# groupeLIAMG/ttcr

Hardware: AMD Instinct MI355X
Metric: Mnodes/s per sweep-iteration (512^3 fp32 grid, first-order FSM) (higher is better)
Workload: dtype f32

## Files before the change

### include/ttcr_amd.h

```cpp
#ifndef TTCR_AMD_H
#define TTCR_AMD_H

#include <stddef.h>
#include <stdint.h>

#ifdef __cplusplus
extern "C" {
#endif

typedef struct ttcr_fsm_grid ttcr_fsm_grid;

enum { TTCR_F32 = 0, TTCR_F64 = 1 };

enum {
    TTCR_OK = 0,
    TTCR_ERR_VALUE = 1,
    TTCR_ERR_RUNTIME = 2,
    TTCR_ERR_DEVICE = 3,
    TTCR_ERR_UNSUPPORTED = 4
};

int ttcr_fsm_device_count(void);

const char* ttcr_fsm_last_error(void);
// ... 200 lines not shown
    double total_ms;
    long long kernel_launches;
    long long node_updates;
    long long evaluated_updates;
    int iterations;
    int n_sources;
} ttcr_fsm_timing;
int ttcr_fsm_last_timing(const ttcr_fsm_grid* g, ttcr_fsm_timing* out);
int ttcr_fsm_stopping_stats(const ttcr_fsm_grid* g, long long* reference_sums, long long* reference_sums_missed, long long* rounds);
int ttcr_fsm_prefill_swaps(const ttcr_fsm_grid* g, long long* swaps);
int ttcr_fsm_prefill_inline_fills(const ttcr_fsm_grid* g, long long* fills);
int ttcr_fsm_reference_change(ttcr_fsm_grid* g, const void* times, const void* field, int parallel, void* out);
int ttcr_fsm_last_kernel(const ttcr_fsm_grid* g, char* buf, size_t n);
int ttcr_fsm_unit_order(int dim, int dtype, int stage, int by_time, uint32_t nnx, uint32_t nny, uint32_t nnz, uint32_t* out,
                        size_t capacity, size_t* n_units);
int ttcr_fsm_prefill_slice(int dtype, uint64_t n_el, uint32_t n_tickets, uint32_t ticket, uint64_t* slice_len, uint64_t* begin, uint64_t* end);
const char* ttcr_fsm_build_id(void);

#ifdef __cplusplus
}
#endif
#endif
```

### ttcr_amd/_lib.py

```python
import ctypes as C
import os

HERE = os.path.dirname(os.path.abspath(__file__))
LIB_PATH = os.environ.get("TTCR_AMD_LIB") or os.path.join(HERE, "libttcr_amd.so")

TTCR_F32, TTCR_F64 = 0, 1
OK, ERR_VALUE, ERR_RUNTIME, ERR_DEVICE, ERR_UNSUPPORTED = 0, 1, 2, 3, 4

_P = C.c_void_p
_U32 = C.c_uint32
_D = C.c_double
_I = C.c_int


class Timing(C.Structure):
    _fields_ = [("sweep_ms", C.c_double), ("total_ms", C.c_double), ("kernel_launches", C.c_longlong),
                ("node_updates", C.c_longlong), ("evaluated_updates", C.c_longlong), ("iterations", C.c_int),
                ("n_sources", C.c_int)]


SYMBOLS = {
    "ttcr_fsm_device_count": (_I, []),
    "ttcr_fsm_last_error": (C.c_char_p, []),
    "ttcr_fsm3d_create": (_I, [C.POINTER(_P), _I, _I, _U32, _U32, _U32, _D, _D, _D, _D, _D, _I, _I, _I, _I, _I]),
# ... 15 lines not shown
    "ttcr_fsm_compute_slowness": (_I, [_P, _I, _P, _I, _P]),
    "ttcr_fsm_get_niter": (_I, [_P, _I, C.POINTER(_I), C.POINTER(_I)]),
    "ttcr_fsm_get_changes": (_I, [_P, _I, C.POINTER(_D), _I, C.POINTER(_D), _I]),
    "ttcr_fsm_get_reference_changes": (_I, [_P, _I, C.POINTER(_D), _I, C.POINTER(_D), _I]),
    "ttcr_fsm_n_slots": (_I, [_P]),
    "ttcr_fsm_n_nodes": (C.c_size_t, [_P]),
    "ttcr_fsm_n_cells": (C.c_size_t, [_P]),
    "ttcr_fsm_set_option": (_I, [_P, C.c_char_p, _D]),
    "ttcr_fsm_last_timing": (_I, [_P, C.POINTER(Timing)]),
    "ttcr_fsm_last_kernel": (_I, [_P, C.c_char_p, C.c_size_t]),
    "ttcr_fsm_build_id": (C.c_char_p, []),
    "ttcr_fsm_unit_order": (_I, [_I, _I, _I, _I, _U32, _U32, _U32, C.POINTER(_U32), C.c_size_t, C.POINTER(C.c_size_t)]),
    "ttcr_fsm_stopping_stats": (_I, [_P, C.POINTER(C.c_longlong), C.POINTER(C.c_longlong), C.POINTER(C.c_longlong)]),
    "ttcr_fsm_prefill_swaps": (_I, [_P, C.POINTER(C.c_longlong)]),
    "ttcr_fsm_prefill_inline_fills": (_I, [_P, C.POINTER(C.c_longlong)]),
    "ttcr_fsm_prefill_slice": (_I, [_I, C.c_uint64, _U32, _U32, C.POINTER(C.c_uint64), C.POINTER(C.c_uint64), C.POINTER(C.c_uint64)]),
    "ttcr_fsm_reference_change": (_I, [_P, C.c_void_p, C.c_void_p, C.c_int, C.c_void_p]),
    "ttcr_fsm_rays_size": (_I, [_P, C.POINTER(C.c_size_t), C.POINTER(C.c_size_t)]),
    "ttcr_fsm_get_rays": (_I, [_P, _P, _P]),
    "ttcr_fsm_raytrace_rays": (_I, [_P, _I, _I, _P, _P, _I, _P, _P]),
    "ttcr_fsm_slot_rays_size": (_I, [_P, _I, C.POINTER(C.c_size_t), C.POINTER(C.c_size_t)]),
    "ttcr_fsm_get_slot_rays": (_I, [_P, _I, _P, _P]),
    "ttcr_fsm_raytrace_m": (_I, [_P, _I, _I, _P, _P, _I, _P, _P]),
    "ttcr_fsm_raytrace_rm": (_I, [_P, _I, _I, _P, _P, _I, _P, _P]),
    "ttcr_fsm_raytrace_multi_m": (_I, [_P, _I, _P, _P, _P, _P, _P, _P, _I]),
    "ttcr_fsm_multi_m_size": (_I, [_P, C.POINTER(C.c_size_t), C.POINTER(C.c_size_t)]),
    "ttcr_fsm_get_multi_m": (_I, [_P, _P, _P, _P]),
    "ttcr_fsm_raytrace_multi_tape": (_I, [_P, _I, _P, _P, _P, _P, _P, _P, C.POINTER(_P)]),
    "ttcr_fsm_tape_size": (_I, [_P, C.POINTER(C.c_size_t), C.POINTER(C.c_size_t), C.POINTER(C.c_size_t)]),
    "ttcr_fsm_tape_bytes": (_I, [_P, C.POINTER(C.c_size_t)]),
# ... 134 lines not shown
```

### ttcr_amd/build.py

```python
import os
import shutil
import subprocess

HERE = os.path.dirname(os.path.abspath(__file__))
CSRC = os.path.join(HERE, "csrc")
OBJ = os.path.join(CSRC, "_obj")
LIB = os.path.join(HERE, "libttcr_amd.so")
INC = os.path.join("..", "..", "include", "ttcr_amd.h")
UNITS = {
    "fsm_capi.hip": ([], ["fsm_capi.hip", "fsm_kernels.h", "fsm_fast_api.h", "fsm_march_levels.inc", "fsm_fast.hip", "fsm_tape_api.h",
                          "fsm_tape.hip", "fsm_adjoint_api.h", "fsm_adjoint.hip", "fsm_normal.hip", "fsm_locate.hip", "fsm_model.hip", "fsm_unit_order.h", "fsm_prefill_slices.h", INC]),
    "fsm_fast.hip": ([], ["fsm_fast.hip", "fsm_fast_api.h", "fsm_kernels.h", "fsm_march_levels.inc", "fsm_prefill_slices.h"]),
    "fsm_tape.hip": ([], ["fsm_tape.hip", "fsm_tape_api.h"]),
    "fsm_adjoint.hip": ([], ["fsm_adjoint.hip", "fsm_adjoint_api.h", "fsm_kernels.h", "fsm_march_levels.inc", "fsm_prefill_slices.h"]),
    "fsm_normal.hip": ([], ["fsm_normal.hip", "fsm_adjoint_api.h"]),
    "fsm_locate.hip": ([], ["fsm_locate.hip", "fsm_adjoint_api.h"]),
    "fsm_model.hip": ([], ["fsm_model.hip", "fsm_adjoint_api.h"]),
}
SOURCES = list(UNITS)
DEPS = sorted({d for _, ds in UNITS.values() for d in ds})
FLAGS = ["--offload-arch=gfx950", "-O3", "-std=c++17", "-fPIC", "-ffp-contract=off",
         "-fno-fast-math", "-Wall", "-Wno-unused-result"]


def _hipcc():
    for c in (os.environ.get("HIPCC"), shutil.which("hipcc"), "/opt/rocm/bin/hipcc"):
        if c and os.path.exists(c):
            return c
    raise RuntimeError("hipcc not found")
# ... 53 lines not shown
```

### ttcr_amd/csrc/fsm_capi.hip

```cpp
#include <hip/hip_runtime.h>

#include <algorithm>
#include <atomic>
#include <chrono>
#include <condition_variable>
#include <cmath>
#include <cstdio>
#include <cstdlib>
#include <cstring>
#include <limits>
#include <map>
#include <memory>
#include <mutex>
#include <sstream>
#include <stdexcept>
#include <string>
#include <thread>
#include <vector>

#include "../../include/ttcr_amd.h"
#include "fsm_kernels.h"
#include "fsm_fast_api.h"
#include "fsm_tape_api.h"
#include "fsm_adjoint_api.h"
#include "fsm_unit_order.h"

#ifndef FSM_CHUNK3
#define FSM_CHUNK3 8
#endif

namespace ttcr_amd {

static thread_local std::string g_last_error;

struct ValueError : std::runtime_error {
    using std::runtime_error::runtime_error;
};
struct DeviceError : std::runtime_error {
    using std::runtime_error::runtime_error;
};
// ... 253 lines not shown
    size_t ssh_stride = 0;
    DevBuf<uint32_t> d_mask;
    DevBuf<int> d_bbox, d_slots, d_lmask;
    int* h_lmask = nullptr;
    DevBuf<uint32_t> d_tiles;
    std::vector<int> tile_off, tile_cnt;
    DevBuf<double> d_change;
    DevBuf<unsigned long long> d_prof;
    size_t prof_words = 0;
    DevBuf<uint32_t> d_order;
    DevBuf<uint32_t> d_order_xs[2][2];
    DevBuf<int> d_sync;
    int n_patches = 0;
    int* h_abort = nullptr;
    DevBuf<int> d_stamp;
    DevBuf<unsigned long long> d_cmap;
    int cmap_words = 1;
    DevBuf<unsigned long long> d_sw;
    int sw_sweeps = 0;
    DevBuf<int> d_iter;
    DevBuf<unsigned long long> d_evals;
    int* h_iter = nullptr;
    unsigned launch_epoch = 1;
    bool sync_clean = true;
    size_t sync_words = 0;
    unsigned long long* h_evals = nullptr;
    int nbf = 0, nbj = 0, nbk = 0;
    size_t n_bricks = 0;
    DevBuf<InitPoint<T>> d_pts;
    double* h_change = nullptr;
// ... 108 lines not shown
        HIP_CHECK(hipMemsetAsync(d_ssh.p, 0, ssh_stride * (dim == 3 ? 4 : 2) * sizeof(T), stream));
        if (dim == 3) build_tile_lists(TileCfg<T, 3>::PJ, TileCfg<T, 3>::PK, TileCfg<T, 3>::BL);
        else build_tile_lists(TileCfg<T, 2>::PJ, TileCfg<T, 2>::PK, TileCfg<T, 2>::BL);
        build_persistent_lists();
        nbf = (geom.NF + FSM_BRICK - 1) / FSM_BRICK;
        nbj = (geom.NJ + FSM_BRICK - 1) / FSM_BRICK;
        nbk = (geom.NK + FSM_BRICK - 1) / FSM_BRICK;
        n_bricks = (size_t)nbf * nbj * nbk;
        d_stamp.reserve(n_bricks * n_slots);
        {
            const int PJ = dim == 3 ? TileCfg<T, 3>::PJ : TileCfg<T, 2>::PJ, PK = dim == 3 ? TileCfg<T, 3>::PK : 1;
            const int max_chunks = (geom.NF + 2 * (PJ + PK)) / 4 + 4;
            cmap_words = max_chunks / 32 + 1;
            d_cmap.reserve((size_t)n_patches * n_slots * (dim == 3 ? 8 : 4) * 2 * cmap_words);
            HIP_CHECK(hipMemset(d_cmap.p, 0, (size_t)n_patches * n_slots * (dim == 3 ? 8 : 4) * 2 * cmap_words * sizeof(unsigned long long)));
            sw_sweeps = (dim == 3 ? 8 : 4) * (2 * std::min(nitermax, 256) + 2);
            d_sw.reserve((size_t)sw_sweeps * n_slots);
        }
        d_iter.reserve(2);
        d_evals.reserve(n_slots);
        if (dim == 2)
            HIP_CHECK(hipFuncSetAttribute(reinterpret_cast<const void*>(&fsm_sweep45_rows<T>),
                                          hipFuncAttributeMaxDynamicSharedMemorySize, 156 * 1024));
        if (const char* e = std::getenv("TTCR_FSM_SWEEP45")) sweep45_strips = std::string(e) == "strips";
        if (const char* e = std::getenv("TTCR_FSM_WENO_CH4_MIN")) weno_ch4_min = std::atoi(e);
        if (const char* e = std::getenv("TTCR_FSM_WENO_C16_BELOW")) weno_c16_below = std::atoi(e);
        if (const char* e = std::getenv("TTCR_FSM_F64_C16_BELOW")) f64_c16_below = std::atoi(e);
        if (const char* e = std::getenv("TTCR_FSM_TIME_ORDER_BELOW")) time_order_below = std::atoi(e);
        if (const char* e = std::getenv("TTCR_FSM_PRE_MIN")) pre_min = std::atoi(e);
        if (const char* e = std::getenv("TTCR_FSM_SKIP")) skip = std::atoi(e);
// ... 73 lines not shown
        a.w = 0;
        a.variant = DIM == 3 ? 0 : (dx == dz ? 1 : 2);
        pa.order = d_order.p;
        pa.sync = d_sync.p;
        pa.n_patches = n_patches;
        pa.batch = batch;
        pa.timeout_ticks = 300000000ull;
        pa.stamp = d_stamp.p;
        pa.iter_ptr = d_iter.p;
        pa.evals = d_evals.p;
        pa.nbf = nbf; pa.nbj = nbj; pa.nbk = nbk;
        pa.ndir = DIM == 3 ? 8 : 4;
        pa.skip = skip_now(batch) ? (std::getenv("TTCR_FSM_SKIP_ALL_DIRTY") ? 2 : 1) : 0;
        pa.cmap = d_cmap.p;
        pa.cw = cmap_words;
        pa.sw = std::getenv("TTCR_FSM_NO_SW") ? nullptr : d_sw.p;
        pa.n_sw_groups = n_groups();
        pa.n_sw_sweeps = sw_sweeps;
        pa.fill_dst = nullptr;
        pa.fill_slice = 0;
        pa.fill_n = 0;

        const size_t wg_cap = (fsm_looped(DIM == 3, H) && persist_wgs > 0) ? (size_t)persist_wgs : ~(size_t)0;
        const dim3 block(C::PJ * C::PK), grid((unsigned)std::min<size_t>((size_t)n_patches * batch, wg_cap));
        const int ndir = DIM == 3 ? 8 : 4;
        {
            const bool pre_ = mode == 2 && !NO_PRE && (DIM == 2 || batch >= pre_min || dyn_lds > 0);
            char nm[160];
            std::snprintf(nm, sizeof nm, "fsm_sweep_persistent<%s,%d,%d,%d,%s,%s,%d,%d,%s,%s>", sizeof(T) == 4 ? "float" : "double", C::PJ, C::PK, CH,
                          DIM == 3 ? "true" : "false", skip_now(batch) ? "true" : "false", H, NSV, mode == 2 ? "true" : "false", pre_ ? "true" : "false");
// ... 327 lines not shown
                if (tile_cnt[w] == 0) continue;
                a.w = w;
                a.tiles = d_tiles.p + tile_off[w];
                const dim3 grid(tile_cnt[w], 1, batch);
                fsm_sweep_tile<T, C::PJ, C::PK, C::BL, DIM == 3><<<grid, block, 0, stream>>>(a);
            }
        }
        last_kernel = std::string("fsm_sweep_tile<") + (sizeof(T) == 4 ? "float" : "double") + "," + std::to_string(C::PJ) + "," + std::to_string(C::PK) + "," + std::to_string(C::BL) + "," + (DIM == 3 ? "true" : "false") + ">";
        HIP_CHECK(hipGetLastError());
    }

    int NS = 1;
    bool ns_window = false;
    int pair_layout = -1;
    double last_eval_frac = -1;
    double layout_lo = 0.55, layout_hi = 0.70;
    void choose_layout() {
        if (!ns_window) return;
        int want = NS;
        if (pair_layout >= 0) want = pair_layout ? 2 : 1;
        else if (last_eval_frac >= 0) want = NS == 2 ? (last_eval_frac < layout_lo ? 1 : 2) : (last_eval_frac > layout_hi ? 2 : 1);
        if (want == NS) return;
        NS = want;
        graph_batches[0] = graph_batches[1] = -1;
        for (int q = 0; q < n_slots; ++q) phys[q] = q;
    }
    int n_groups() const { return (n_slots + NS - 1) / NS; }
    size_t tt_fields() const { return (size_t)n_slots + ((ns_window || NS == 2) ? (size_t)(n_slots & 1) : 0); }
    T* tt_ptr(int slot) const { return d_tt.p + (size_t)(slot / NS) * n_nodes * NS + slot % NS; }
    template <int H>
    bool fast_now() const { return sizeof(T) == 4 && (arith == 2 || (arith == 1 && !weno)); }
// ... 19 lines not shown
    int skip_probe_min = 1024;
    bool probe_skip = true;
    int probe_off_calls = 0;
    int persist_wgs = 2048;
    bool in_probe_window(int entries) const {
        const long long u = (long long)n_patches * entries;
        return dim == 3 && sizeof(T) == 4 && u >= skip_probe_min && u < skip_units_min;
    }
    int skip_default(int entries) const {
        if (dim != 3) return 1;
        if (stage == 1) return 1;
        if (in_probe_window(entries)) return probe_skip ? 1 : 0;
        return (long long)n_patches * entries >= skip_units_min ? 1 : 0;
    }
    bool persistent_now() const { return mode >= 1 || stage == 1; }
    bool skip_now(int entries) const {
        const int on = skip < 0 ? skip_default(entries) : skip;
        const bool fits = (long long)geom.NF + geom.NJ + geom.NK < (1ll << 22) && nbf <= 32 * FSM_SLAB_WORDS;
        return on != 0 && fits && !(dim == 2 && rotated && !weno && dx == dz);
    }

    void launch_sweep45(int batch) {
        Sweep45Args<T> a;
        a.tt = d_tt.p;
        a.s = d_s.p;
        a.frozen = d_mask.p;
        a.change = d_change.p;
        a.slots = d_slots.p;
        a.lmask = d_lmask.p;
        a.ts = NS;
        a.by_group = persistent_now() ? 1 : 0;
        a.nnx = (int)ncx + 1;
        a.nnz = (int)ncz + 1;
// ... 436 lines not shown

        const int maxit = fixed_iters > 0 ? fixed_iters : nitermax;
        const int ndir = dim == 3 ? 8 : 4;
        if (!sync_clean || launch_epoch > 0xfffff000u) {
            HIP_CHECK(hipMemsetAsync(d_sync.p, 0, sync_words * sizeof(int), stream));
            HIP_CHECK(hipMemsetAsync(d_cmap.p, 0, (size_t)n_patches * n_slots * ndir * 2 * cmap_words * sizeof(unsigned long long), stream));
            HIP_CHECK(hipStreamSynchronize(stream));
            launch_epoch = 1;
        }
        sync_clean = false;
        snap_always = false;
        if (persistent_now() || weno) HIP_CHECK(hipMemsetAsync(d_sync.p + 8, 0, (sync_words - 8) * sizeof(int), stream));
        if (persistent_now() || weno) HIP_CHECK(hipMemsetAsync(d_sync.p + 4, 0, sizeof(int), stream));
        HIP_CHECK(hipMemsetAsync(d_evals.p, 0, sizeof(unsigned long long) * n_slots, stream));
        HIP_CHECK(hipMemsetAsync(d_sw.p, 0, sizeof(unsigned long long) * (size_t)sw_sweeps * n_groups(), stream));
        HIP_CHECK(hipEventRecord(ev0, stream));
        int it_total = 0;
        for (stage = 0; stage < (weno ? 2 : 1); ++stage) {
            std::vector<int> active(slot_ids);
            int it = 0;
            prev_change.assign(n_slots, std::numeric_limits<double>::infinity());
            prev2_change.assign(n_slots, std::numeric_limits<double>::infinity());
            snap_iter.assign(n_groups(), 0);
            snap_T.assign(n_groups(), -1);
            stamps_ok = false;
            if ((int)ref_change_last.size() != n_slots) ref_change_last.assign(n_slots, std::nan(""));
            std::vector<int> groups;
            for (int s2 : slot_ids)
                if (groups.empty() || groups.back() != s2 / NS) groups.push_back(s2 / NS);
            while (!active.empty() && it < maxit) {
// ... 3200 lines not shown
        } else {
            PJ = dim == 3 ? TileCfg<double, 3>::PJ : TileCfg<double, 2>::PJ; PK = dim == 3 ? TileCfg<double, 3>::PK : 1;
            C = dim == 3 ? ChunkCfg<double, 3>::C : ChunkCfg<double, 2>::C;
        }
        const uint64_t npj = ((uint64_t)NJ + PJ - 1) / PJ, npk = ((uint64_t)NK + PK - 1) / PK;
        if (NF >= (1u << 30) || npj >= (1u << 14) || npk >= (1u << 14)) throw ValueError("grid too large for the patch index of the sweep kernel");
        *n_units = (size_t)(npj * npk) * (dim == 3 ? 8 : 4);
        if (!out) return;
        if (capacity < *n_units) throw ValueError("output buffer too small for the units of the launch");
        const std::vector<uint32_t> xs = fsm_xs_order(dim, (int)NF, (int)NJ, (int)NK, PJ, PK, C, stage == 0 ? 1 : 2, by_time != 0,
                                                      fsm_diag_order((int)npj, (int)npk));
        std::copy(xs.begin(), xs.end(), out);
    });
}

int ttcr_fsm_prefill_slice(int dtype, uint64_t n_el, uint32_t n_tickets, uint32_t ticket, uint64_t* slice_len, uint64_t* begin, uint64_t* end) {
    return guarded([&] {
        if (dtype != TTCR_F32 && dtype != TTCR_F64) throw ValueError("dtype must be TTCR_F32 or TTCR_F64");
        if (n_tickets == 0) throw ValueError("a launch has at least one ticket");
        const size_t slice = fsm_fill_slice_len((size_t)n_el, n_tickets, dtype == TTCR_F32 ? 4 : 2);
        size_t b = 0, e = 0;
        fsm_fill_slice_range((size_t)n_el, slice, ticket, &b, &e);
        if (slice_len) *slice_len = slice;
        if (begin) *begin = b;
        if (end) *end = e;
    });
}

const char* ttcr_fsm_build_id(void) { return TTCR_BUILD_ID; }

// ... 2 lines not shown
```

### ttcr_amd/csrc/fsm_kernels.h

```cpp
#pragma once
#include <hip/hip_runtime.h>
#include <stdint.h>
#include <type_traits>

#include "fsm_prefill_slices.h"

namespace ttcr_amd {

constexpr int FSM_BRICK = 16;

template <typename T> struct real_traits;
template <> struct real_traits<float> {
    static __host__ __device__ constexpr float max() { return 3.402823466e+38f; }
    static __device__ __forceinline__ float inf() { return __builtin_huge_valf(); }
};
template <> struct real_traits<double> {
    static __host__ __device__ constexpr double max() { return 1.7976931348623157e+308; }
    static __device__ __forceinline__ double inf() { return __builtin_huge_val(); }
};

__device__ __forceinline__ uint32_t idx_u32(double v) { return v < 0 ? 0u : (v >= 4294967295.0 ? 4294967295u : (uint32_t)v); }

__device__ __forceinline__ float rmin(float a, float b) { return a < b ? a : b; }
__device__ __forceinline__ double rmin(double a, double b) { return a < b ? a : b; }
// ... 405 lines not shown
    SweepArgs<T> s;
    const uint32_t* order;
    int* sync;
    int n_patches, batch;
    unsigned long long timeout_ticks;
    int* stamp;
    const int* iter_ptr;
    unsigned long long* evals;
    int nbf, nbj, nbk;
    int dir, ndir;
    int skip;
    unsigned long long* cmap;
    int cw;
    unsigned long long* sw;
    int n_sw_groups, n_sw_sweeps;
    const T* ssh;
    size_t ssh_stride;
    T* fill_dst;
    size_t fill_slice;
    size_t fill_n;
};



__device__ __forceinline__ float ld_sc1(const float* p) {
    return __uint_as_float(__hip_atomic_load((const unsigned int*)p, __ATOMIC_RELAXED, __HIP_MEMORY_SCOPE_AGENT));
}
__device__ __forceinline__ double ld_sc1(const double* p) {
    return __longlong_as_double(__hip_atomic_load((const long long*)p, __ATOMIC_RELAXED, __HIP_MEMORY_SCOPE_AGENT));
}
// ... 238 lines not shown
    const float disc3 = __builtin_fmaf(3.0f * fh, fh, -(df2 + __builtin_fmaf(d3, d3, e * e)));
    const float t3 = __builtin_fmaf(1.0f / 3.0f, (d3 - df) + __builtin_amdgcn_sqrtf(disc3), a1);
    return t1 > a2 ? (t2 > a3 ? t3 : t2) : t1;
}

#ifndef FSM_POLL_SLEEP
#define FSM_POLL_SLEEP 2
#endif
#ifndef FSM_MINW
#define FSM_MINW 1
#endif
#ifndef FSM_SLAB_WORDS
#define FSM_SLAB_WORDS 32
#endif
#define FSM_FIN 0x3ffffff0
#ifndef FSM_SKIP_ABL
#define FSM_SKIP_ABL 0
#endif
#ifndef FSM_EARLY_PUB
#define FSM_EARLY_PUB 0
#endif
__device__ __forceinline__ float lane_below(float x, float edge) {
    return __uint_as_float((unsigned)__builtin_amdgcn_update_dpp((int)__float_as_uint(edge), (int)__float_as_uint(x), 0x138, 0xf, 0xf, false));
}
__device__ __forceinline__ float lane_above(float x, float edge) {
    return __uint_as_float((unsigned)__builtin_amdgcn_update_dpp((int)__float_as_uint(edge), (int)__float_as_uint(x), 0x130, 0xf, 0xf, false));
}
__device__ __forceinline__ double lane_below(double x, double edge) {
    const unsigned long long u = (unsigned long long)__double_as_longlong(x), e = (unsigned long long)__double_as_longlong(edge);
    const unsigned lo = (unsigned)__builtin_amdgcn_update_dpp((int)(unsigned)e, (int)(unsigned)u, 0x138, 0xf, 0xf, false);
// ... 39 lines not shown
    const unsigned long long u = (unsigned long long)__float_as_uint(x.v[0]) | ((unsigned long long)__float_as_uint(x.v[1]) << 32);
    __hip_atomic_store((unsigned long long*)p, u, __ATOMIC_RELAXED, __HIP_MEMORY_SCOPE_AGENT);
}
__device__ __forceinline__ void st_sc1(Pack<double, 2>* p, Pack<double, 2> x) {
    st_sc1(&p->v[0], x.v[0]);
    st_sc1(&p->v[1], x.v[1]);
}

__host__ __device__ constexpr bool fsm_looped(bool is3d, int h) { return is3d && h == 1; }

__device__ __forceinline__ int kmaxp_of(int k0, int NK, int PK) { return (k0 + PK < NK ? k0 + PK : NK) - 1; }
template <typename T, int PJ, int PK, int C, bool IS3D, bool SKIP, int H, int NS, bool XS, bool PRE, int AR = 0>
__device__ __forceinline__ bool fsm_sweep_unit(const PersistArgs<T>& pa) {
    static_assert(AR == 0 || std::is_same<T, float>::value, "tolerance-grade arithmetic: fp32 kernels");
    constexpr bool LOOPED = fsm_looped(IS3D, H);
    using P = Pack<T, NS>;
    constexpr int NT = PJ * PK;
    constexpr int RJ = PJ + 2 * H;
    constexpr int NROWS = IS3D ? RJ * (PK + 2 * H) : RJ;
    constexpr int NQ = C + 2 * H;
    constexpr int RS = NQ | 1;
    constexpr int NUP = IS3D ? H * (PJ + PK) : H;
    constexpr int NDH = IS3D ? H * (PJ + PK) : H;
    constexpr int RPI = NT / C;
    constexpr int NOWN = C;
    constexpr int NHI = (NDH + RPI - 1) / RPI;
    constexpr int NUPI = (NUP + RPI - 1) / RPI;
    static_assert(NT % C == 0 && (IS3D || PK == 1) && C <= FSM_BRICK && (H == 1 || H == 2), "tile shape");
    static_assert(C - 1 <= FSM_XPAD, "the rows of a chunk are read from the sheared copies without a wrap");
    static_assert(!(SKIP && FSM_EARLY_PUB > 0), "FSM_EARLY_PUB is a tuning option of the kernels without exact skipping");
// ... 7 lines not shown
        __hip_atomic_store(p_, (int)(((unsigned)e2 << 30) | (unsigned)v_), __ATOMIC_RELAXED, __HIP_MEMORY_SCOPE_AGENT);
    };
    auto ld_cmap = [&](const unsigned long long* p_) -> unsigned {
        const unsigned long long v_ = __hip_atomic_load(p_, __ATOMIC_RELAXED, __HIP_MEMORY_SCOPE_AGENT);
        return (unsigned)(v_ >> 32) == epoch ? (unsigned)v_ : 0u;
    };
    auto st_cmap = [&](unsigned long long* p_, unsigned v_) {
        __hip_atomic_store(p_, ((unsigned long long)epoch << 32) | v_, __ATOMIC_RELAXED, __HIP_MEMORY_SCOPE_AGENT);
    };

    __shared__ P Tt[NROWS * RS];
    __shared__ int s_ticket, s_abort;
    __shared__ int s_anychg;
    constexpr int SLABW = SKIP ? FSM_SLAB_WORDS : 1;
    __shared__ unsigned s_stamped[SKIP ? 9 : 1][SLABW];
    __shared__ unsigned s_slab[SLABW];
    __shared__ int s_next, s_act;
    __shared__ int s_cwi[2], s_cwl[2];
    __shared__ unsigned s_cwv[2];
    __shared__ int s_mywi;
    __shared__ unsigned s_mywv[2];
    enum { U_THR, U_RSJLO, U_RSKLO, U_RSNJ, U_RSNK, U_LCF, U_UPLCF0, U_UPLCF1, U_HIST, U_EVER, U_UCHG, U_PENDV, U_LCHG, U_N };
    __shared__ int s_u[U_N];

    int tid = threadIdx.x;
    if constexpr (LOOPED) asm volatile("" : "+v"(tid));
    unsigned long long prof_t = (FSM_ENABLE_PROF && a.prof) ? wall_clock64() : 0ull;
    unsigned long long pacc[6] = {0, 0, 0, 0, 0, 0};
    unsigned pchunks = 0;
    unsigned long long twait = 0;
    constexpr int FSM_TRACE_UNITS = FSM_ENABLE_PROF == 2 ? (1 << 20) : 65536;
    const unsigned long long trace_t0 = prof_t;
    unsigned long long* prec = nullptr;
    __shared__ unsigned long long s_pacc[FSM_ENABLE_PROF == 2 ? 8 : 1];
    if constexpr (FSM_ENABLE_PROF == 2) {
        if (tid == 0) {
            for (int q = 0; q < 6; ++q) s_pacc[q] = 0;
            s_pacc[6] = prof_t;
// ... 368 lines not shown
                        if (__hip_atomic_load(pa.sync + 4, __ATOMIC_RELAXED, __HIP_MEMORY_SCOPE_AGENT)) break;
                        if (wall_clock64() - t0 > pa.timeout_ticks) {
                            __hip_atomic_store(pa.sync + 4, 1, __ATOMIC_RELAXED, __HIP_MEMORY_SCOPE_AGENT);
                            break;
                        }
                    }
                    __builtin_amdgcn_s_sleep(8);
                }
            }
        }
        __syncthreads();
    }
    if (CHASE_OK && chase) chase_wait(Lc - C, -1, false);
    if (!SKIP) { issue_static(Lc); pref_for = Lc; }
    if constexpr (SKIP) {
        const int nsw = (pa.nbf + 31) >> 5;
        for (int w = tid; w < nsw; w += NT) s_slab[w] = 0u;
        for (int w = tid; w < 9 * SLABW; w += NT) s_stamped[w / SLABW][w % SLABW] = 0u;
        if (tid == 0) {
            s_cwi[0] = -1; s_cwi[1] = -1; s_mywi = -1;
            const int ja = j0 - H < 0 ? 0 : j0 - H, jb = jmaxp + H > NJ - 1 ? NJ - 1 : jmaxp + H;
            const int ka = k0 - H < 0 ? 0 : k0 - H, kb = kmaxp + H > NK - 1 ? NK - 1 : kmaxp + H;
            const int jlo = (rj ? NJ - 1 - jb : ja) / FSM_BRICK, jhi = (rj ? NJ - 1 - ja : jb) / FSM_BRICK;
            const int klo = (rk ? NK - 1 - kb : ka) / FSM_BRICK, khi = (rk ? NK - 1 - ka : kb) / FSM_BRICK;
            s_u[U_RSJLO] = jlo; s_u[U_RSNJ] = jhi - jlo + 1;
            s_u[U_RSKLO] = klo; s_u[U_RSNK] = khi - klo + 1;
            const int sg = pa.ndir * pa.iter_ptr[0] + dir + 1;
            s_u[U_THR] = pa.skip == 2 ? -(1 << 30) : (sg - 1 > 0 ? sg - 1 : 0);
            s_u[U_LCF] = Lc;
            const int lsj = Ls - PJ, lsk = Ls - PK, mu = TJ + TK - 1;
            s_u[U_UPLCF0] = lsj - (((lsj - mu) % C + C) % C);
            s_u[U_UPLCF1] = lsk - (((lsk - mu) % C + C) % C);
            s_u[U_HIST] = 0; s_u[U_EVER] = 0; s_u[U_UCHG] = 0; s_u[U_PENDV] = 0; s_u[U_LCHG] = 0;
        }
        __syncthreads();
        {
            const int jlo = s_u[U_RSJLO], nj = s_u[U_RSNJ], klo = s_u[U_RSKLO], nk = s_u[U_RSNK], thr = s_u[U_THR];
            const int* __restrict__ stamp = pa.stamp + (size_t)grp * pa.nbf * pa.nbj * pa.nbk;
            const int total = pa.nbf * nj * nk;
            for (int b = tid; b < total; b += NT) {
                const int bf = b % pa.nbf, jk = b / pa.nbf;
                const int bj = jlo + jk % nj, bk = klo + jk / nj;
                const int v = __hip_atomic_load(stamp + ((size_t)bk * pa.nbj + bj) * pa.nbf + bf, __ATOMIC_RELAXED, __HIP_MEMORY_SCOPE_AGENT);
                if (v >= thr) atomicOr(&s_slab[bf >> 5], 1u << (bf & 31));
            }
        }
        __syncthreads();
    }
    FSM_PMARK(5)
    const unsigned long long trace_t1 = (FSM_ENABLE_PROF && a.prof) ? wall_clock64() : 0ull;
    auto cmap_of = [&](int pidx, int e) -> unsigned long long* {
// ... 80 lines not shown
                        const int need8 = (L + C - 1) << 8;
                        bool ok = true;
                        if (up_j && pre_j < need8) pre_j = poll_until(up_j, need8, ok);
                        if (up_k && ok && pre_k < need8) pre_k = poll_until(up_k, need8, ok);
                        if (!ok) act = 0;
                        break;
                    }
                    const int need = L + C - 1, need8 = need << 8;
                    int vj = FSM_FIN, vk = FSM_FIN;
                    bool ok = true;
                    if (up_j) { vj = pre_j >= need8 ? pre_j : poll_until(up_j, need8, ok); pre_j = vj; }
                    if (up_k && ok) { vk = pre_k >= need8 ? pre_k : poll_until(up_k, need8, ok); pre_k = vk; }
                    if (!ok) { act = 0; break; }
                    if (L == lcf && vj >= FSM_FIN && !(vj & 1) && vk >= FSM_FIN && !(vk & 2)) {
                        bool any = false;
                        for (int w = 0; w < ((pa.nbf + 31) >> 5); ++w) any |= s_slab[w] != 0u;
                        if (!any) {
                            st_prog(my_prog, FSM_FIN);
                            L = Le + 1;
                            act = 0;
                            break;
                        }
                    }
                    int flo, fhi;
                    chunk_frange(L, H, flo, fhi);
                    bool dirty = slab_any(flo, fhi);
                    if (!dirty && up_j) dirty = up_dirty(vj, need, 0);
                    if (!dirty && up_k) dirty = up_dirty(vk, need, 1);
                    if (dirty) break;
                    if (pending) { act = 2; break; }
                    L += C;
                    h = (h << 2) & 0xff;
                    if (L > Le && s_u[U_UCHG]) {
                        s_u[U_PENDV] = FSM_FIN | s_u[U_EVER];
                    } else {
                        st_prog(my_prog, L > Le ? (FSM_FIN | s_u[U_EVER]) : ((L << 8) | h));
                    }
                }
                s_u[U_HIST] = h;
                s_next = L;
                s_act = act;
// ... 176 lines not shown
        FSM_PMARK(3)
        if (FSM_ENABLE_PROF) ++pchunks;

        if constexpr (SKIP) {
            const bool ej = changed && jp + H > jmaxp, ek = IS3D && changed && kp + H > kmaxp;
            const int f = (wave_any(changed) ? 1 : 0) | (wave_any(ej) ? 2 : 0) | (wave_any(ek) ? 4 : 0);
            if (f && (tid & 63) == 0) atomicOr(&s_anychg, f);
            if (!(FSM_SKIP_ABL & 2) && changed) {
                const int ip0 = L0 - jp - kp;
                const int ia = ip0 + ea, ib = ip0 + eb;
                const int ba = (rf ? NF - 1 - ib : ia) / FSM_BRICK, bb2 = (rf ? NF - 1 - ia : ib) / FSM_BRICK;
                const int my_bj = (rj ? NJ - 1 - jp : jp) / FSM_BRICK - s_u[U_RSJLO], my_bk = (rk ? NK - 1 - kp : kp) / FSM_BRICK - s_u[U_RSKLO];
                const int jk = my_bk * s_u[U_RSNJ] + my_bj;
                atomicOr(&s_stamped[jk][ba >> 5], 1u << (ba & 31));
                if (bb2 != ba) atomicOr(&s_stamped[jk][bb2 >> 5], 1u << (bb2 & 31));
            }
        } else {
            if (wave_any(changed) && (tid & 63) == 0) s_anychg = 1;
        }
        __syncthreads();
        const int chg_flags = SKIP ? __builtin_amdgcn_readfirstlane(s_anychg) : s_anychg;
        const bool any_changed = chg_flags != 0;
        if (any_changed) {
#pragma unroll
            for (int it = 0; it < NOWN; ++it) {
                const int ipm = L0 + ipb[it] - H;
                if ((unsigned)ipm < (unsigned)NF) {
                    const int rid = rsub + RPI * it;
                    const int cj = rid % PJ, ck = rid / PJ;
                    P* dst = Tg + (abase[it] + sf * (L0 - H));
                    const P v = Tt[lrow[it] - H];
                    if (XS || cj >= PJ - H || (IS3D && ck >= PK - H)) st_sc1(dst, v); else *dst = v;
                }
            }
        }
        if constexpr (SKIP) {
            if (!(FSM_SKIP_ABL & 4) && tid == 0) {
                if (any_changed) {
                    int flo, fhi;
                    chunk_frange(L0, 0, flo, fhi);
                    for (int b = flo / FSM_BRICK; b <= fhi / FSM_BRICK; ++b) s_slab[b >> 5] |= 1u << (b & 31);
                    const int ci = (L0 - s_u[U_LCF]) / C, w = ci >> 5;
                    if ((chg_flags & 6) && w < pa.cw) {
                        if (s_mywi != w) { s_mywi = w; s_mywv[0] = 0u; s_mywv[1] = 0u; }
                        for (int e2 = 0; e2 < 2; ++e2)
                            if (chg_flags & (2 << e2)) {
                                s_mywv[e2] |= 1u << (ci & 31);
                                st_cmap(cmap_of(TK * npj + TJ, e2) + w, s_mywv[e2]);
                            }
                    }
                    s_u[U_UCHG] = 1;
                    s_u[U_LCHG] = 1;
                }
                const int h2 = ((s_u[U_HIST] << 2) | (chg_flags >> 1)) & 0xff, ev2 = s_u[U_EVER] | (chg_flags >> 1);
                s_u[U_HIST] = h2;
                s_u[U_EVER] = ev2;
                s_u[U_PENDV] = Lc + C > Le ? (FSM_FIN | ev2) : (((Lc + C) << 8) | h2);
            }
        }
// ... 8 lines not shown
        ++n_done;
        FSM_PMARK(4)
    }
    if constexpr (SKIP) {
        __syncthreads();
        if (s_u[U_UCHG]) {
            const int nsw = (pa.nbf + 31) >> 5;
            const int rs_jlo = s_u[U_RSJLO], rs_nj = s_u[U_RSNJ], rs_klo = s_u[U_RSKLO], njk = rs_nj * s_u[U_RSNK];
            int* __restrict__ stamp = pa.stamp + (size_t)grp * pa.nbf * pa.nbj * pa.nbk;
            const int sigma = pa.ndir * pa.iter_ptr[0] + dir + 1;
            for (int q = tid; q < njk * nsw * 32; q += NT) {
                const int jk = q / (nsw * 32), bf = q % (nsw * 32);
                if (bf < pa.nbf && ((s_stamped[jk][bf >> 5] >> (bf & 31)) & 1u))
                    atomicMax(stamp + ((size_t)(rs_klo + jk / rs_nj) * pa.nbj + rs_jlo + jk % rs_nj) * pa.nbf + bf, sigma);
            }
            pending = 1;
        }
    }
    if (pending) {
        asm volatile("s_waitcnt vmcnt(0)" ::: "memory");
        __syncthreads();
        if (tid == 0) st_prog(my_prog, SKIP ? s_u[U_PENDV] : pending);
    }
    if constexpr (SKIP) {
        const int sigma0 = pa.ndir * pa.iter_ptr[0] + dir;
        if (tid == 0 && pa.sw && sigma0 < pa.n_sw_sweeps)
            atomicAdd(pa.sw + (size_t)sigma0 * pa.n_sw_groups + grp, 1ull | (s_u[U_UCHG] ? (1ull << 32) : 0ull));
    }

    if (FSM_ENABLE_PROF && a.prof && tid == 0) {
// ... 22 lines not shown
    for (int l = 0; l < NS; ++l) {
        double accd = (double)dec[l];
#pragma unroll
        for (int off = 32; off > 0; off >>= 1) accd += __shfl_down(accd, off, 64);
        if ((tid & 63) == 0 && accd != 0.0) atomicAdd(a.change + grp * NS + l, accd);
        if ((tid & 63) == 0 && nevals && ((lm >> l) & 1)) atomicAdd(pa.evals + grp * NS + l, nevals);
    }
    return true;
}

template <typename T, int PJ, int PK, int C, bool IS3D, bool SKIP, int H, int NS, bool XS, bool PRE = false, int AR = 0>
#ifndef FSM_WENO_MINW
#define FSM_WENO_MINW FSM_MINW
#endif
__global__ __launch_bounds__(PJ* PK, (SKIP && IS3D && H == 1 && NS == 2 && sizeof(T) == 4) ? 3
                                     : (IS3D && H == 2 && NS == 1 && sizeof(T) == 4) ? FSM_WENO_MINW : FSM_MINW) void fsm_sweep_persistent(const PersistArgs<T> pa) {
    if constexpr (fsm_looped(IS3D, H)) {
        (void)pa;
        for (;;) {
            auto kp = __builtin_amdgcn_kernarg_segment_ptr();
            asm volatile("" : "+s"(kp));
            if (!fsm_sweep_unit<T, PJ, PK, C, IS3D, SKIP, H, NS, XS, PRE, AR>(*(const PersistArgs<T>*)kp)) break;
        }
    } else {
        fsm_sweep_unit<T, PJ, PK, C, IS3D, SKIP, H, NS, XS, PRE, AR>(pa);
    }
}

template <typename T>
struct Sweep45Args {
// ... 1772 lines not shown
```

Measured before the change: 95910.

## Track per-chunk dirty bits for next sweep direction instead of brick slab scan

Adds a per-patch, per-direction chunk dirty bitmap. Each tile writes the chunks of neighbouring tiles that its updated nodes affect in the next sweep direction, and reads its own bitmap to decide which level chunks to skip. This replaces the per-chunk scan of brick stamps and slab bits with a single bit lookup, and also retunes the layout switch thresholds. In exchange it adds shared-memory arrays, atomic ORs to global memory, and extra register pressure, with a lower occupancy bound for the fp64 variant.

```diff
diff --git a/include/ttcr_amd.h b/include/ttcr_amd.h
--- a/include/ttcr_amd.h
+++ b/include/ttcr_amd.h
@@ -238,6 +238,7 @@
 int ttcr_fsm_last_kernel(const ttcr_fsm_grid* g, char* buf, size_t n);
 int ttcr_fsm_unit_order(int dim, int dtype, int stage, int by_time, uint32_t nnx, uint32_t nny, uint32_t nnz, uint32_t* out,
                         size_t capacity, size_t* n_units);
+int ttcr_fsm_chunk_dirty_marks(int dtype, int chunk, int dir, int edge_rule, uint32_t nnx, uint32_t nny, uint32_t nnz, int32_t* out, size_t capacity);
 int ttcr_fsm_prefill_slice(int dtype, uint64_t n_el, uint32_t n_tickets, uint32_t ticket, uint64_t* slice_len, uint64_t* begin, uint64_t* end);
 const char* ttcr_fsm_build_id(void);
 
diff --git a/ttcr_amd/_lib.py b/ttcr_amd/_lib.py
--- a/ttcr_amd/_lib.py
+++ b/ttcr_amd/_lib.py
@@ -53,6 +53,7 @@
     "ttcr_fsm_stopping_stats": (_I, [_P, C.POINTER(C.c_longlong), C.POINTER(C.c_longlong), C.POINTER(C.c_longlong)]),
     "ttcr_fsm_prefill_swaps": (_I, [_P, C.POINTER(C.c_longlong)]),
     "ttcr_fsm_prefill_inline_fills": (_I, [_P, C.POINTER(C.c_longlong)]),
+    "ttcr_fsm_chunk_dirty_marks": (_I, [_I, _I, _I, _I, _U32, _U32, _U32, C.POINTER(C.c_int32), C.c_size_t]),
     "ttcr_fsm_prefill_slice": (_I, [_I, C.c_uint64, _U32, _U32, C.POINTER(C.c_uint64), C.POINTER(C.c_uint64), C.POINTER(C.c_uint64)]),
     "ttcr_fsm_reference_change": (_I, [_P, C.c_void_p, C.c_void_p, C.c_int, C.c_void_p]),
     "ttcr_fsm_rays_size": (_I, [_P, C.POINTER(C.c_size_t), C.POINTER(C.c_size_t)]),
diff --git a/ttcr_amd/build.py b/ttcr_amd/build.py
--- a/ttcr_amd/build.py
+++ b/ttcr_amd/build.py
@@ -9,10 +9,10 @@
 INC = os.path.join("..", "..", "include", "ttcr_amd.h")
 UNITS = {
     "fsm_capi.hip": ([], ["fsm_capi.hip", "fsm_kernels.h", "fsm_fast_api.h", "fsm_march_levels.inc", "fsm_fast.hip", "fsm_tape_api.h",
-                          "fsm_tape.hip", "fsm_adjoint_api.h", "fsm_adjoint.hip", "fsm_normal.hip", "fsm_locate.hip", "fsm_model.hip", "fsm_unit_order.h", "fsm_prefill_slices.h", INC]),
-    "fsm_fast.hip": ([], ["fsm_fast.hip", "fsm_fast_api.h", "fsm_kernels.h", "fsm_march_levels.inc", "fsm_prefill_slices.h"]),
+                          "fsm_tape.hip", "fsm_adjoint_api.h", "fsm_adjoint.hip", "fsm_normal.hip", "fsm_locate.hip", "fsm_model.hip", "fsm_unit_order.h", "fsm_prefill_slices.h", "fsm_chunk_dirty.h", INC]),
+    "fsm_fast.hip": ([], ["fsm_fast.hip", "fsm_fast_api.h", "fsm_kernels.h", "fsm_march_levels.inc", "fsm_prefill_slices.h", "fsm_chunk_dirty.h"]),
     "fsm_tape.hip": ([], ["fsm_tape.hip", "fsm_tape_api.h"]),
-    "fsm_adjoint.hip": ([], ["fsm_adjoint.hip", "fsm_adjoint_api.h", "fsm_kernels.h", "fsm_march_levels.inc", "fsm_prefill_slices.h"]),
+    "fsm_adjoint.hip": ([], ["fsm_adjoint.hip", "fsm_adjoint_api.h", "fsm_kernels.h", "fsm_march_levels.inc", "fsm_prefill_slices.h", "fsm_chunk_dirty.h"]),
     "fsm_normal.hip": ([], ["fsm_normal.hip", "fsm_adjoint_api.h"]),
     "fsm_locate.hip": ([], ["fsm_locate.hip", "fsm_adjoint_api.h"]),
     "fsm_model.hip": ([], ["fsm_model.hip", "fsm_adjoint_api.h"]),
diff --git a/ttcr_amd/csrc/fsm_capi.hip b/ttcr_amd/csrc/fsm_capi.hip
--- a/ttcr_amd/csrc/fsm_capi.hip
+++ b/ttcr_amd/csrc/fsm_capi.hip
@@ -24,6 +24,7 @@
 #include "fsm_tape_api.h"
 #include "fsm_adjoint_api.h"
 #include "fsm_unit_order.h"
+#include "fsm_chunk_dirty.h"
 
 #ifndef FSM_CHUNK3
 #define FSM_CHUNK3 8
@@ -307,6 +308,7 @@
     int n_patches = 0;
     int* h_abort = nullptr;
     DevBuf<int> d_stamp;
+    DevBuf<unsigned> d_cdirty;
     DevBuf<unsigned long long> d_cmap;
     int cmap_words = 1;
     DevBuf<unsigned long long> d_sw;
@@ -445,6 +447,8 @@
             cmap_words = max_chunks / 32 + 1;
             d_cmap.reserve((size_t)n_patches * n_slots * (dim == 3 ? 8 : 4) * 2 * cmap_words);
             HIP_CHECK(hipMemset(d_cmap.p, 0, (size_t)n_patches * n_slots * (dim == 3 ? 8 : 4) * 2 * cmap_words * sizeof(unsigned long long)));
+            cdirty_wpu = ((geom.NF + 2 * (PJ + PK)) / 8 + 4) / 32 + 1;
+            if (dim == 3) d_cdirty.reserve(cdirty_words());
             sw_sweeps = (dim == 3 ? 8 : 4) * (2 * std::min(nitermax, 256) + 2);
             d_sw.reserve((size_t)sw_sweeps * n_slots);
         }
@@ -548,6 +552,8 @@
         pa.skip = skip_now(batch) ? (std::getenv("TTCR_FSM_SKIP_ALL_DIRTY") ? 2 : 1) : 0;
         pa.cmap = d_cmap.p;
         pa.cw = cmap_words;
+        pa.cdirty = d_cdirty.p;
+        pa.cdw = cdirty_wpu;
         pa.sw = std::getenv("TTCR_FSM_NO_SW") ? nullptr : d_sw.p;
         pa.n_sw_groups = n_groups();
         pa.n_sw_sweeps = sw_sweeps;
@@ -905,7 +911,7 @@
     bool ns_window = false;
     int pair_layout = -1;
     double last_eval_frac = -1;
-    double layout_lo = 0.55, layout_hi = 0.70;
+    double layout_lo = 0.45, layout_hi = 0.55;
     void choose_layout() {
         if (!ns_window) return;
         int want = NS;
@@ -955,9 +961,11 @@
         return (long long)n_patches * entries >= skip_units_min ? 1 : 0;
     }
     bool persistent_now() const { return mode >= 1 || stage == 1; }
+    int cdirty_wpu = 1;
+    size_t cdirty_words() const { return (size_t)n_patches * n_slots * 8 * cdirty_wpu; }
     bool skip_now(int entries) const {
         const int on = skip < 0 ? skip_default(entries) : skip;
-        const bool fits = (long long)geom.NF + geom.NJ + geom.NK < (1ll << 22) && nbf <= 32 * FSM_SLAB_WORDS;
+        const bool fits = (long long)geom.NF + geom.NJ + geom.NK < (1ll << 22) && nbf <= 32 * FSM_SLAB_WORDS && (dim != 3 || cdirty_wpu <= FSM_CD_WORDS);
         return on != 0 && fits && !(dim == 2 && rotated && !weno && dx == dz);
     }
 
@@ -1424,6 +1432,7 @@
         if (persistent_now() || weno) HIP_CHECK(hipMemsetAsync(d_sync.p + 4, 0, sizeof(int), stream));
         HIP_CHECK(hipMemsetAsync(d_evals.p, 0, sizeof(unsigned long long) * n_slots, stream));
         HIP_CHECK(hipMemsetAsync(d_sw.p, 0, sizeof(unsigned long long) * (size_t)sw_sweeps * n_groups(), stream));
+        if (d_cdirty.p) HIP_CHECK(hipMemsetAsync(d_cdirty.p, 0, cdirty_words() * sizeof(unsigned), stream));
         HIP_CHECK(hipEventRecord(ev0, stream));
         int it_total = 0;
         for (stage = 0; stage < (weno ? 2 : 1); ++stage) {
@@ -4654,6 +4663,33 @@
     });
 }
 
+int ttcr_fsm_chunk_dirty_marks(int dtype, int chunk, int dir, int edge_rule, uint32_t nnx, uint32_t nny, uint32_t nnz, int32_t* out, size_t capacity) {
+    return guarded([&] {
+        if (dtype != TTCR_F32 && dtype != TTCR_F64) throw ValueError("dtype must be TTCR_F32 or TTCR_F64");
+        if (chunk != 8 && chunk != 16) throw ValueError("chunk must be 8 or 16 levels");
+        if (dir < 0 || dir > 7) throw ValueError("dir must be one of the eight sweep directions");
+        if (nnx < 2 || nny < 2 || nnz < 2) throw ValueError("grid needs at least two nodes per axis");
+        if (!out) throw ValueError("null output");
+        const int PJ = dtype == TTCR_F32 ? TileCfg<float, 3>::PJ : TileCfg<double, 3>::PJ, PK = dtype == TTCR_F32 ? TileCfg<float, 3>::PK : TileCfg<double, 3>::PK;
+        const uint64_t n = (uint64_t)nnx * nny * nnz;
+        if (n >= (1ull << 31)) throw ValueError("grid too large");
+        if (capacity < (size_t)n * 12) throw ValueError("output buffer too small: 12 words per node");
+        const int NF = (int)nnx, NJ = (int)nny, NK = (int)nnz, dn = (dir + 1) % 8;
+        for (int k = 0; k < NK; ++k)
+            for (int j = 0; j < NJ; ++j)
+                for (int i = 0; i < NF; ++i) {
+                    int32_t* o = out + (((size_t)k * NJ + j) * NF + i) * 12;
+                    int m = 0;
+                    for (int q = 0; q < 12; ++q) o[q] = -1;
+                    fsm_chunk_marks(NF, NJ, NK, PJ, PK, chunk, 1, dn, j, k, i, i, edge_rule != 0, [&](int tj, int tk, int c0, int c1) {
+                        if (m == 3) throw std::logic_error("ttcr_fsm_chunk_dirty_marks: a node marks more than three units");
+                        o[4 * m] = tj; o[4 * m + 1] = tk; o[4 * m + 2] = c0; o[4 * m + 3] = c1;
+                        ++m;
+                    });
+                }
+    });
+}
+
 int ttcr_fsm_prefill_slice(int dtype, uint64_t n_el, uint32_t n_tickets, uint32_t ticket, uint64_t* slice_len, uint64_t* begin, uint64_t* end) {
     return guarded([&] {
         if (dtype != TTCR_F32 && dtype != TTCR_F64) throw ValueError("dtype must be TTCR_F32 or TTCR_F64");
diff --git a/ttcr_amd/csrc/fsm_chunk_dirty.h b/ttcr_amd/csrc/fsm_chunk_dirty.h
--- /dev/null
+++ b/ttcr_amd/csrc/fsm_chunk_dirty.h
@@ -0,0 +1,50 @@
+#pragma once
+
+#if defined(__HIPCC__) || defined(__CUDACC__)
+#define FSM_CD_HD __host__ __device__ __forceinline__
+#else
+#define FSM_CD_HD inline
+#endif
+
+FSM_CD_HD int fsm_chunk_first(int TJ, int TK, int PJ, int PK, int C) {
+    const int Ls = TJ * PJ + TK * PK;
+    return Ls - (((Ls - (TJ + TK)) % C + C) % C);
+}
+
+template <class Emit>
+FSM_CD_HD void fsm_chunk_mark_units(int NF, int NJ, int NK, int PJ, int PK, int C, int H, int dn, int jn, int kn, bool edge_rule, Emit&& emit) {
+    const int rj = (dn >> 1) & 1, rk = (dn >> 2) & 1;
+    const int j2 = rj ? NJ - 1 - jn : jn, k2 = rk ? NK - 1 - kn : kn;
+    const int TJ = j2 / PJ, TK = k2 / PK;
+    auto one = [&](int tj, int tk) {
+        const int j0 = tj * PJ, k0 = tk * PK;
+        const int jm = (j0 + PJ < NJ ? j0 + PJ : NJ) - 1, km = (k0 + PK < NK ? k0 + PK : NK) - 1;
+        const int lcf = fsm_chunk_first(tj, tk, PJ, PK, C);
+        emit(tj, tk, lcf - (j2 + k2), (jm + km + NF - 1 - lcf) / C + 1);
+    };
+    one(TJ, TK);
+    if (edge_rule) {
+        if (TJ > 0 && j2 - H < TJ * PJ) one(TJ - 1, TK);
+        if ((TJ + 1) * PJ < NJ && j2 + H >= (TJ + 1) * PJ) one(TJ + 1, TK);
+        if (TK > 0 && k2 - H < TK * PK) one(TJ, TK - 1);
+        if ((TK + 1) * PK < NK && k2 + H >= (TK + 1) * PK) one(TJ, TK + 1);
+    }
+}
+
+FSM_CD_HD bool fsm_chunk_mark_range(int NF, int C, int dn, int rel, int nch, int fa, int fb, int* c0, int* c1) {
+    const int rf = dn & 1;
+    const int ia = (rf ? NF - 1 - fb : fa) - 1 - rel, ib = (rf ? NF - 1 - fa : fb) + 1 - rel;
+    const int a = ia < 0 ? 0 : ia / C, b = ib < 0 ? -1 : (ib / C < nch - 1 ? ib / C : nch - 1);
+    *c0 = a;
+    *c1 = b;
+    return a <= b;
+}
+
+template <class Emit>
+FSM_CD_HD void fsm_chunk_marks(int NF, int NJ, int NK, int PJ, int PK, int C, int H, int dn, int jn, int kn, int fa, int fb,
+                               bool edge_rule, Emit&& emit) {
+    fsm_chunk_mark_units(NF, NJ, NK, PJ, PK, C, H, dn, jn, kn, edge_rule, [&](int tj, int tk, int rel, int nch) {
+        int c0, c1;
+        if (fsm_chunk_mark_range(NF, C, dn, rel, nch, fa, fb, &c0, &c1)) emit(tj, tk, c0, c1);
+    });
+}
diff --git a/ttcr_amd/csrc/fsm_kernels.h b/ttcr_amd/csrc/fsm_kernels.h
--- a/ttcr_amd/csrc/fsm_kernels.h
+++ b/ttcr_amd/csrc/fsm_kernels.h
@@ -3,6 +3,7 @@
 #include <stdint.h>
 #include <type_traits>
 
+#include "fsm_chunk_dirty.h"
 #include "fsm_prefill_slices.h"
 
 namespace ttcr_amd {
@@ -443,6 +444,8 @@
     int cw;
     unsigned long long* sw;
     int n_sw_groups, n_sw_sweeps;
+    unsigned* cdirty;
+    int cdw;
     const T* ssh;
     size_t ssh_stride;
     T* fill_dst;
@@ -711,6 +714,10 @@
 #define FSM_SLAB_WORDS 32
 #endif
 #define FSM_FIN 0x3ffffff0
+#ifndef FSM_CHUNK_DIRTY
+#define FSM_CHUNK_DIRTY 1
+#endif
+#define FSM_CD_WORDS (2 * FSM_SLAB_WORDS + 4)
 #ifndef FSM_SKIP_ABL
 #define FSM_SKIP_ABL 0
 #endif
@@ -780,6 +787,8 @@
 __device__ __forceinline__ bool fsm_sweep_unit(const PersistArgs<T>& pa) {
     static_assert(AR == 0 || std::is_same<T, float>::value, "tolerance-grade arithmetic: fp32 kernels");
     constexpr bool LOOPED = fsm_looped(IS3D, H);
+    constexpr bool CD = FSM_CHUNK_DIRTY && SKIP && IS3D && H == 1;
+    static_assert(!CD || C >= 8, "the host sizes the dirty bits for chunks of 8 levels or more");
     using P = Pack<T, NS>;
     constexpr int NT = PJ * PK;
     constexpr int RJ = PJ + 2 * H;
@@ -817,14 +826,18 @@
     __shared__ int s_anychg;
     constexpr int SLABW = SKIP ? FSM_SLAB_WORDS : 1;
     __shared__ unsigned s_stamped[SKIP ? 9 : 1][SLABW];
-    __shared__ unsigned s_slab[SLABW];
+    __shared__ unsigned s_slab[CD ? 1 : SLABW];
+    constexpr int CDW = CD ? FSM_CD_WORDS : 1;
+    __shared__ unsigned s_cd[CDW];
+    __shared__ int s_cmp[CD ? 3 * NT : 1], s_cml[CD ? 3 * NT : 1];
+    __shared__ unsigned s_mark[9 * CDW];
     __shared__ int s_next, s_act;
     __shared__ int s_cwi[2], s_cwl[2];
     __shared__ unsigned s_cwv[2];
     __shared__ int s_mywi;
     __shared__ unsigned s_mywv[2];
-    enum { U_THR, U_RSJLO, U_RSKLO, U_RSNJ, U_RSNK, U_LCF, U_UPLCF0, U_UPLCF1, U_HIST, U_EVER, U_UCHG, U_PENDV, U_LCHG, U_N };
-    __shared__ int s_u[U_N];
+    enum { U_THR, U_RSJLO, U_RSKLO, U_RSNJ, U_RSNK, U_LCF, U_UPLCF0, U_UPLCF1, U_HIST, U_EVER, U_UCHG, U_PENDV, U_LCHG, U_MKJ0, U_MKK0 };
+    __shared__ int s_u[CD ? U_MKK0 + 1 : U_MKJ0];
 
     int tid = threadIdx.x;
     if constexpr (LOOPED) asm volatile("" : "+v"(tid));
@@ -1223,8 +1236,10 @@
     if (CHASE_OK && chase) chase_wait(Lc - C, -1, false);
     if (!SKIP) { issue_static(Lc); pref_for = Lc; }
     if constexpr (SKIP) {
-        const int nsw = (pa.nbf + 31) >> 5;
-        for (int w = tid; w < nsw; w += NT) s_slab[w] = 0u;
+        if constexpr (!CD) {
+            const int nsw = (pa.nbf + 31) >> 5;
+            for (int w = tid; w < nsw; w += NT) s_slab[w] = 0u;
+        }
         for (int w = tid; w < 9 * SLABW; w += NT) s_stamped[w / SLABW][w % SLABW] = 0u;
         if (tid == 0) {
             s_cwi[0] = -1; s_cwi[1] = -1; s_mywi = -1;
@@ -1241,9 +1256,54 @@
             s_u[U_UPLCF0] = lsj - (((lsj - mu) % C + C) % C);
             s_u[U_UPLCF1] = lsk - (((lsk - mu) % C + C) % C);
             s_u[U_HIST] = 0; s_u[U_EVER] = 0; s_u[U_UCHG] = 0; s_u[U_PENDV] = 0; s_u[U_LCHG] = 0;
+            if constexpr (CD) {
+                const int dn = (dir + 1) % pa.ndir;
+                const int fj = rj != ((dn >> 1) & 1), fk = rk != ((dn >> 2) & 1);
+                const int ja2 = (fj ? NJ - 1 - jmaxp : j0) - H, ka2 = (fk ? NK - 1 - kmaxp : k0) - H;
+                s_u[U_MKJ0] = (ja2 < 0 ? 0 : ja2) / PJ;
+                s_u[U_MKK0] = (ka2 < 0 ? 0 : ka2) / PK;
+            }
+        }
+        if constexpr (CD) {
+            unsigned* cdw = pa.cdirty + ((((size_t)grp * pa.ndir + dir) * pa.n_patches) + (size_t)(TK * npj + TJ)) * pa.cdw;
+            const bool first_sweep = pa.iter_ptr[0] == 0 && dir == 0;
+            for (int w = tid; w < pa.cdw && w < CDW; w += NT) {
+                unsigned v = pa.skip == 2 ? 0xffffffffu : __hip_atomic_exchange(cdw + w, 0u, __ATOMIC_RELAXED, __HIP_MEMORY_SCOPE_AGENT);
+                if (first_sweep) {
+                    const int jlo = (rj ? NJ - 1 - jmaxp : j0) - 1, jhi = (rj ? NJ - 1 - j0 : jmaxp) + 1;
+                    const int klo = (rk ? NK - 1 - kmaxp : k0) - 1, khi = (rk ? NK - 1 - k0 : kmaxp) + 1;
+#pragma unroll 1
+                    for (int l = 0; l < NS; ++l) {
+                        const int* b6 = bb + 6 * l;
+                        if (jhi < b6[2] || jlo > b6[3] || khi < b6[4] || klo > b6[5]) continue;
+                        const int b0 = (rf ? NF - 1 - b6[1] : b6[0]) - 1, b1 = (rf ? NF - 1 - b6[0] : b6[1]) + 1;
+                        int ca = b0 + j0 + k0 - Lc, cb = b1 + jmaxp + kmaxp - Lc;
+                        if (cb < 0) continue;
+                        ca = (ca < 0 ? 0 : ca / C) - 32 * w;
+                        cb = cb / C - 32 * w;
+                        if (cb < 0 || ca > 31) continue;
+                        v |= (ca <= 0 ? 0xffffffffu : 0xffffffffu << ca) & (cb >= 31 ? 0xffffffffu : (2u << cb) - 1u);
+                    }
+                }
+                s_cd[w] = v;
+            }
+            for (int w = tid; w < 9 * pa.cdw && w < 9 * CDW; w += NT) s_mark[w] = 0u;
         }
         __syncthreads();
-        {
+        if constexpr (CD) {
+            int q = 0;
+            const int mj0 = s_u[U_MKJ0], mk0 = s_u[U_MKK0];
+            if (col_ok)
+                fsm_chunk_mark_units(NF, NJ, NK, PJ, PK, C, H, (dir + 1) % pa.ndir, jn, kn, true, [&](int tj_, int tk_, int rel, int nch) {
+                    const int pj = tj_ - mj0, pk = tk_ - mk0;
+                    if (q >= 3 || (unsigned)pj >= 3u || (unsigned)pk >= 3u) return;
+                    s_cmp[q * NT + tid] = (pk * 3 + pj) | (nch << 4);
+                    s_cml[q * NT + tid] = rel;
+                    ++q;
+                });
+            for (; q < 3; ++q) s_cmp[q * NT + tid] = -1;
+        }
+        if constexpr (!CD) {
             const int jlo = s_u[U_RSJLO], nj = s_u[U_RSNJ], klo = s_u[U_RSKLO], nk = s_u[U_RSNK], thr = s_u[U_THR];
             const int* __restrict__ stamp = pa.stamp + (size_t)grp * pa.nbf * pa.nbj * pa.nbk;
             const int total = pa.nbf * nj * nk;
@@ -1354,7 +1414,11 @@
                     if (!ok) { act = 0; break; }
                     if (L == lcf && vj >= FSM_FIN && !(vj & 1) && vk >= FSM_FIN && !(vk & 2)) {
                         bool any = false;
-                        for (int w = 0; w < ((pa.nbf + 31) >> 5); ++w) any |= s_slab[w] != 0u;
+                        if constexpr (CD) {
+                            for (int w = 0; w < pa.cdw; ++w) any |= s_cd[w] != 0u;
+                        } else {
+                            for (int w = 0; w < ((pa.nbf + 31) >> 5); ++w) any |= s_slab[w] != 0u;
+                        }
                         if (!any) {
                             st_prog(my_prog, FSM_FIN);
                             L = Le + 1;
@@ -1362,9 +1426,15 @@
                             break;
                         }
                     }
-                    int flo, fhi;
-                    chunk_frange(L, H, flo, fhi);
-                    bool dirty = slab_any(flo, fhi);
+                    bool dirty;
+                    if constexpr (CD) {
+                        const int ci = (L - lcf) / C;
+                        dirty = (s_cd[ci >> 5] >> (ci & 31)) & 1u;
+                    } else {
+                        int flo, fhi;
+                        chunk_frange(L, H, flo, fhi);
+                        dirty = slab_any(flo, fhi);
+                    }
                     if (!dirty && up_j) dirty = up_dirty(vj, need, 0);
                     if (!dirty && up_k) dirty = up_dirty(vk, need, 1);
                     if (dirty) break;
@@ -1571,6 +1641,25 @@
                 const int jk = my_bk * s_u[U_RSNJ] + my_bj;
                 atomicOr(&s_stamped[jk][ba >> 5], 1u << (ba & 31));
                 if (bb2 != ba) atomicOr(&s_stamped[jk][bb2 >> 5], 1u << (bb2 & 31));
+                if constexpr (CD) {
+                    const int fa = rf ? NF - 1 - ib : ia, fb = rf ? NF - 1 - ia : ib, cw = pa.cdw, dn = (dir + 1) % pa.ndir;
+#pragma unroll 1
+                    for (int q = 0; q < 3; ++q) {
+                        const int pn = s_cmp[q * NT + tid];
+                        int c0, c1;
+                        if (pn < 0 || !fsm_chunk_mark_range(NF, C, dn, s_cml[q * NT + tid], pn >> 4, fa, fb, &c0, &c1)) continue;
+                        unsigned* mrow = s_mark + (pn & 15) * cw;
+                        const int w0 = c0 >> 5, w1 = c1 >> 5;
+                        const unsigned m0 = ~0u << (c0 & 31), m1 = (2u << (c1 & 31)) - 1u;
+                        if (w1 >= cw || w1 >= CDW) continue;
+                        if (w0 == w1) {
+                            atomicOr(mrow + w0, m0 & m1);
+                        } else {
+                            atomicOr(mrow + w0, m0);
+                            atomicOr(mrow + w1, m1);
+                        }
+                    }
+                }
             }
         } else {
             if (wave_any(changed) && (tid & 63) == 0) s_anychg = 1;
@@ -1594,12 +1683,18 @@
         if constexpr (SKIP) {
             if (!(FSM_SKIP_ABL & 4) && tid == 0) {
                 if (any_changed) {
-                    int flo, fhi;
-                    chunk_frange(L0, 0, flo, fhi);
-                    for (int b = flo / FSM_BRICK; b <= fhi / FSM_BRICK; ++b) s_slab[b >> 5] |= 1u << (b & 31);
+                    if constexpr (!CD) {
+                        int flo, fhi;
+                        chunk_frange(L0, 0, flo, fhi);
+                        for (int b = flo / FSM_BRICK; b <= fhi / FSM_BRICK; ++b) s_slab[b >> 5] |= 1u << (b & 31);
+                    }
                     const int ci = (L0 - s_u[U_LCF]) / C, w = ci >> 5;
                     if ((chg_flags & 6) && w < pa.cw) {
-                        if (s_mywi != w) { s_mywi = w; s_mywv[0] = 0u; s_mywv[1] = 0u; }
+                        if (s_mywi != w) {
+                            unsigned z0 = 0u;
+                            if constexpr (CD) asm volatile("" : "+v"(z0));
+                            s_mywi = w; s_mywv[0] = z0; s_mywv[1] = z0;
+                        }
                         for (int e2 = 0; e2 < 2; ++e2)
                             if (chg_flags & (2 << e2)) {
                                 s_mywv[e2] |= 1u << (ci & 31);
@@ -1638,6 +1733,15 @@
                 if (bf < pa.nbf && ((s_stamped[jk][bf >> 5] >> (bf & 31)) & 1u))
                     atomicMax(stamp + ((size_t)(rs_klo + jk / rs_nj) * pa.nbj + rs_jlo + jk % rs_nj) * pa.nbf + bf, sigma);
             }
+            if constexpr (CD) {
+                const int cw = pa.cdw, mj0 = s_u[U_MKJ0], mk0 = s_u[U_MKK0], npk = a.g.npk;
+                unsigned* cdn = pa.cdirty + (((size_t)grp * pa.ndir + (dir + 1) % pa.ndir) * pa.n_patches) * cw;
+                for (int q = tid; q < 9 * cw && q < 9 * CDW; q += NT) {
+                    const unsigned v = s_mark[q];
+                    const int p9 = q / cw, tj_ = mj0 + p9 % 3, tk_ = mk0 + p9 / 3;
+                    if (v && tj_ < npj && tk_ < npk) atomicOr(cdn + (size_t)(tk_ * npj + tj_) * cw + q % cw, v);
+                }
+            }
             pending = 1;
         }
     }
@@ -1690,6 +1794,7 @@
 #define FSM_WENO_MINW FSM_MINW
 #endif
 __global__ __launch_bounds__(PJ* PK, (SKIP && IS3D && H == 1 && NS == 2 && sizeof(T) == 4) ? 3
+                                     : (FSM_CHUNK_DIRTY && SKIP && IS3D && H == 1 && NS == 2 && sizeof(T) == 8) ? 2
                                      : (IS3D && H == 2 && NS == 1 && sizeof(T) == 4) ? FSM_WENO_MINW : FSM_MINW) void fsm_sweep_persistent(const PersistArgs<T> pa) {
     if constexpr (fsm_looped(IS3D, H)) {
         (void)pa;
```

Measured after the change: 99350, median of 6. 1.04x the previous value.
